# lhoyer/improving_segmentation_with_selfsupervised_depth

Measured on AMD Instinct MI355X. Metric: train images/sec, ResNet-101 joint seg+depth @512x1024, higher is better.
Workload: dtype f32

## Files before the change

improving_segmentation_with_selfsupervised_depth_amd/_lib.py:

```python
import ctypes
import os
from ctypes import c_int, c_long, c_float, c_void_p, c_size_t, c_uint64, c_int64, POINTER

_HERE = os.path.dirname(os.path.abspath(__file__))
LIB_PATH = os.environ.get("SEGSDE_LIB") or os.path.join(_HERE, "libsegsde_hip.so")
ABI_VERSION = 23

_LIB = None
HOST_POINTERS_OK = False


class PackJob(ctypes.Structure):
    _fields_ = [("w", c_void_p), ("fwd", c_void_p), ("dgrad", c_void_p)] + [(n, c_int) for n in (
        "O", "I", "KH", "KW", "block0", "reserved")]


class WinoJob(ctypes.Structure):
    _fields_ = [("w", c_void_p), ("u_fwd", c_void_p), ("u_dgrad", c_void_p)] + [(n, c_int) for n in ("O", "I", "block0", "reserved")]


class BnFoldJob(ctypes.Structure):
    _fields_ = [(n, c_void_p) for n in ("w", "cb", "gamma", "beta", "mean", "var", "w_out", "b_out")] + [("eps", c_float)] + [
        (n, c_int) for n in ("O", "I", "KH", "KW", "block0", "reserved")]


class ConvDesc(ctypes.Structure):
    _fields_ = [(n, c_int) for n in (
        "B", "H", "W", "C0", "C1", "ld0", "ld1", "up0", "Ho", "Wo", "Cout", "ldy", "ldy2", "nsplit",
        "KH", "KW", "stride", "dil", "pad", "pad_mode", "in_div", "act", "sum2x2", "accumulate", "compute")]
# ... 48 lines not shown
    "segsde_pack_weight_both": (c_int, [P, P, P, c_int, c_int, c_int, c_int, P]),
    "segsde_pack_weight_both_multi": (c_int, [P, c_int, c_int, P]),
    "segsde_reflect_dgrad_fix": (c_int, [P, c_int, P, P, c_int, P, c_int, c_int, c_int, c_int, c_int, c_int, c_int, P]),
    "segsde_bn_stats_workspace": (c_size_t, [c_long, c_int]),
    "segsde_bn_stats": (c_int, [P, c_int, c_long, c_int, P, P, P, P, c_float, c_float, P, P, c_size_t, P]),
    "segsde_bn_eval_stats": (c_int, [P, P, c_int, c_float, P, P, P]),
    "segsde_bn_fold": (c_int, [P, c_int, c_int, P]),
    "segsde_bn_apply": (c_int, [P, c_int, c_long, c_int, P, P, P, P, P, c_int, P, c_int, c_int, c_float, c_uint64, P]),
    "segsde_bn_backward_workspace": (c_size_t, [c_long, c_int]),
    "segsde_bn_backward": (c_int, [P, c_int, P, c_int, P, c_int, c_long, c_int, P, P, P, P, c_int, c_float, c_uint64, c_int,
                                   P, P, P, c_int, P, c_int, P, c_size_t, P]),
    "segsde_bn_mask_words": (c_size_t, [c_long, c_int]),
    "segsde_bn_apply_mask": (c_int, [P, c_int, c_long, c_int, P, P, P, P, P, c_int, P, c_int, c_int, c_float, c_uint64, P, P]),
    "segsde_bn_backward_mask": (c_int, [P, c_int, P, P, c_int, c_long, c_int, P, P, P, c_int, c_float, c_int, P, P, P, c_int, P, c_int,
                                        P, c_size_t, P]),
    "segsde_colsum_workspace": (c_size_t, [c_long, c_int]),
    "segsde_act_backward": (c_int, [P, c_int, P, c_int, c_long, c_int, c_int, P, c_int, P, P, c_size_t, P]),
    "segsde_colsum": (c_int, [P, c_int, c_long, c_int, P, P, c_size_t, P]),
    "segsde_feat_dist_workspace": (c_size_t, [c_long, c_int]),
    "segsde_feat_dist_forward": (c_int, [P, c_int, P, c_int, c_long, c_int, P, P, c_size_t, P]),
    "segsde_feat_dist_backward": (c_int, [P, c_int, P, c_int, c_long, c_int, P, P, P, c_int, P]),
    "segsde_maxpool3x3s2_forward": (c_int, [P, c_int, c_int, c_int, c_int, P, P, P]),
    "segsde_maxpool3x3s2_backward": (c_int, [P, P, c_int, c_int, c_int, c_int, P, c_int, P]),
    "segsde_upsample2x_backward": (c_int, [P, c_int, c_int, c_int, c_int, c_int, P, c_int, P]),
    "segsde_upsample2x_forward": (c_int, [P, c_int, c_int, c_int, c_int, c_int, P, c_int, P]),
    "segsde_resize_bilinear_forward": (c_int, [P, c_int, c_int, c_int, c_int, c_int, P, c_int, c_int, c_int, c_int, P]),
    "segsde_resize_bilinear_backward": (c_int, [P, c_int, c_int, c_int, c_int, c_int, P, c_int, c_int, c_int, c_int, P]),
    "segsde_global_avgpool_workspace": (c_size_t, [c_int, c_long, c_int]),
    "segsde_global_avgpool_forward": (c_int, [P, c_int, c_int, c_long, c_int, P, P, c_size_t, P]),
    "segsde_global_avgpool_backward": (c_int, [P, c_int, c_long, c_int, P, c_int, P]),
    "segsde_gate_forward": (c_int, [P, P, c_long, P, P]),
    "segsde_gate_backward": (c_int, [P, P, P, c_long, P, P, P]),
    "segsde_axpby": (c_int, [c_long, c_float, P, c_float, P, P, P]),
    "segsde_axpby_dev": (c_int, [c_long, P, P, P, P, P, P]),
    "segsde_scale_channels": (c_int, [P, c_int, c_int, c_long, c_int, P, P, c_int, P]),
    "segsde_dropout": (c_int, [P, c_int, c_long, c_int, c_float, c_uint64, P, c_int, P]),
    "segsde_copy_channels": (c_int, [P, c_int, P, c_int, c_long, c_int, P]),
    "segsde_nchw_to_nhwc": (c_int, [P, c_int, c_int, c_int, c_int, c_float, c_float, P, c_int, P]),
    "segsde_nhwc_to_nchw": (c_int, [P, c_int, c_int, c_int, c_int, c_int, P, P]),
    "segsde_pose_matrix_forward": (c_int, [P, P, c_int, c_int, c_int, P, P]),
    "segsde_pose_matrix_backward": (c_int, [P, P, P, c_int, c_int, c_int, P, P, P]),
    "segsde_warp_forward": (c_int, [P, c_int, c_int, P, P, P, P, c_int, c_int, c_int, c_float, c_float, P, P, P, P]),
    "segsde_warp_backward_workspace": (c_size_t, [c_int, c_int, c_int]),
    "segsde_warp_backward": (c_int, [P, P, c_int, c_int, P, P, P, P, c_int, c_int, c_int, c_float, c_float, P, P, P,
                                     c_size_t, P]),
    "segsde_reprojection_error_forward": (c_int, [P, P, c_int, c_int, c_int, c_int, P, c_long, P]),
# ... 99 lines not shown
```

improving_segmentation_with_selfsupervised_depth_amd/csrc/elementwise.hip:

```cpp
#include <stdlib.h>
#include "segsde_common.h"
#include <type_traits>
#include <utility>
#include <cstdlib>
#include <cstring>

namespace {

template <int VW> struct VecF { float v[VW]; };
template <int VW> __device__ __forceinline__ VecF<VW> ldv(const float* p) {
  VecF<VW> r;
  if (VW == 4) { const float4 t = *reinterpret_cast<const float4*>(p); r.v[0] = t.x; r.v[1 % VW] = t.y; r.v[2 % VW] = t.z; r.v[3 % VW] = t.w; }
  else r.v[0] = p[0];
  return r;
}
template <int VW> __device__ __forceinline__ void stv(float* p, const VecF<VW>& r) {
  if (VW == 4) *reinterpret_cast<float4*>(p) = make_float4(r.v[0], r.v[1 % VW], r.v[2 % VW], r.v[3 % VW]);
  else p[0] = r.v[0];
}

constexpr int SLAB = 64;
constexpr int RLANES = 4;

__host__ __device__ inline int red_blocks(long M) {
  long nb = (M + 255) / 256;
  return (int)(nb < 1 ? 1 : (nb > 512 ? 512 : nb));
}

template <class Op, int VW, class = void> struct has_ctx : std::false_type {};
template <class Op, int VW>
struct has_ctx<Op, VW, std::void_t<decltype(std::declval<const Op&>().template ctx<VW>(0))>> : std::true_type {};


template <class Op, int VW, int TX>
__global__ __launch_bounds__(256) void colreduce_kernel(Op op, long M, int C, double* part) {
  constexpr int TY = 256 / TX, CW = TX * VW;
  SEGSDE_SMEM;
  double* sh = reinterpret_cast<double*>(segsde_smem);
  const int tx = threadIdx.x % TX, ty = threadIdx.x / TX;
  const int c = blockIdx.y * CW + tx * VW;
  const int nb = gridDim.x;
  const long rows_per = (M + nb - 1) / nb;
  const long r_begin = blockIdx.x * rows_per;
  long r_end = r_begin + rows_per; if (r_end > M) r_end = M;
  double s0[VW], s1[VW];
#pragma unroll
  for (int j = 0; j < VW; ++j) { s0[j] = 0.0; s1[j] = 0.0; }
  if (c < C) {
    if constexpr (has_ctx<Op, VW>::value) {
      const auto k = op.template ctx<VW>(c);
      for (long m = r_begin + ty; m < r_end; m += TY) op.template row<VW>(m, c, k, s0, s1);
    } else {
#pragma unroll 4
      for (long m = r_begin + ty; m < r_end; m += TY) op.template row<VW>(m, c, s0, s1);
    }
  }
#pragma unroll
  for (int j = 0; j < VW; ++j) {
    sh[ty * CW + tx * VW + j] = s0[j];
    sh[(TY + ty) * CW + tx * VW + j] = s1[j];
  }
  __syncthreads();
  const int cc = threadIdx.x;
  if (cc < CW && blockIdx.y * CW + cc < C) {
    double a = 0.0, b2 = 0.0;
    for (int j = 0; j < TY; ++j) { a += sh[j * CW + cc]; b2 += sh[(TY + j) * CW + cc]; }
    part[((long)blockIdx.x * 2 + 0) * C + blockIdx.y * CW + cc] = a;
    part[((long)blockIdx.x * 2 + 1) * C + blockIdx.y * CW + cc] = b2;
  }
}

template <class Op, int TX>
void launch_colreduce_scalar(Op op, long M, int C, double* part, hipStream_t s) {
  const dim3 grid(red_blocks(M), (C + TX - 1) / TX);
// ... 373 lines not shown
    const int w = t % W; t /= W;
    const int h = t % H; const int b = t / H;
    float4 s = make_float4(0.f, 0.f, 0.f, 0.f);
    for (int kh = 0; kh < 3; ++kh) {
      const int hn = h + 1 - kh;
      if (hn < 0 || (hn & 1)) continue;
      const int ho = hn >> 1; if (ho >= Ho) continue;
      for (int kw = 0; kw < 3; ++kw) {
        const int wn = w + 1 - kw;
        if (wn < 0 || (wn & 1)) continue;
        const int wo = wn >> 1; if (wo >= Wo) continue;
        const long o = ((long)(b * Ho + ho) * Wo + wo) * C4 + c4;
        const uchar4 k = reinterpret_cast<const uchar4*>(idx)[o];
        const float4 g = reinterpret_cast<const float4*>(dy)[o];
        const unsigned char tap = (unsigned char)(kh * 3 + kw);
        s.x += k.x == tap ? g.x : 0.f; s.y += k.y == tap ? g.y : 0.f; s.z += k.z == tap ? g.z : 0.f; s.w += k.w == tap ? g.w : 0.f;
      }
    }
    if (accumulate) {
      const float4 o = reinterpret_cast<const float4*>(dx)[e];
      s.x += o.x; s.y += o.y; s.z += o.z; s.w += o.w;
    }
    reinterpret_cast<float4*>(dx)[e] = s;
  }
}

__global__ __launch_bounds__(256) void upsample2x_bwd_kernel(const float* dy, int lddy, int B, int h, int w, int C,
                                                             float* dx, int lddx) {
  const long total = (long)B * h * w * C;
  const int W2 = 2 * w;
  for (long e = blockIdx.x * 256L + threadIdx.x; e < total; e += (long)gridDim.x * 256) {
    const int c = (int)(e % C); long t = e / C;
    const int x = (int)(t % w); t /= w;
    const int y = (int)(t % h); const int b = (int)(t / h);
    const float* p = dy + ((long)(b * 2 * h + 2 * y) * W2 + 2 * x) * lddy + c;
    const float s = (p[0] + p[lddy]) + (p[(long)W2 * lddy] + p[(long)W2 * lddy + lddy]);
    dx[((long)(b * h + y) * w + x) * lddx + c] = s;
  }
}

__global__ __launch_bounds__(256) void upsample2x_fwd_kernel(const float* x, int ldx, int B, int h, int w, int C, float* y,
                                                             int ldy) {
  const long total = (long)B * 2 * h * 2 * w * C;
  for (long e = blockIdx.x * 256L + threadIdx.x; e < total; e += (long)gridDim.x * 256) {
    const int c = (int)(e % C); long t = e / C;
    const int X = (int)(t % (2 * w)); t /= 2 * w;
// ... 566 lines not shown
                       C / 4, Ho, Wo, y, idx);
  } else {
    hipLaunchKernelGGL(maxpool_fwd_kernel, dim3(ew_blocks((long)B * Ho * Wo * C)), dim3(256), 0, ST(stream), x, B, H, W, C,
                       Ho, Wo, y, idx);
  }
  SEGSDE_CHECK_LAUNCH();
  return 0;
}
extern "C" int segsde_maxpool3x3s2_backward(const float* dy, const uint8_t* idx, int B, int H, int W, int C, float* dx,
                                            int accumulate, void* stream) {
  if (!dy || !idx || !dx) return SEGSDE_ERR_NULL;
  const int Ho = (H - 1) / 2 + 1, Wo = (W - 1) / 2 + 1;
  if (C % 4 == 0 && (long)B * H * W * (C / 4) < (1L << 31) && al16p(dy) && al16p(dx) && (reinterpret_cast<uintptr_t>(idx) & 3) == 0) {
    hipLaunchKernelGGL(maxpool_bwd4_kernel, dim3(ew_blocks((long)B * H * W * (C / 4))), dim3(256), 0, ST(stream), dy, idx, B, H, W,
                       C / 4, Ho, Wo, dx, accumulate);
    SEGSDE_CHECK_LAUNCH();
    return 0;
  }
  hipLaunchKernelGGL(maxpool_bwd_kernel, dim3(ew_blocks((long)B * H * W * C)), dim3(256), 0, ST(stream), dy, idx, B, H, W,
                     C, Ho, Wo, dx, accumulate);
  SEGSDE_CHECK_LAUNCH();
  return 0;
}
extern "C" int segsde_upsample2x_backward(const float* dy, int lddy, int B, int h, int w, int C, float* dx, int lddx,
                                          void* stream) {
  if (!dy || !dx) return SEGSDE_ERR_NULL;
  hipLaunchKernelGGL(upsample2x_bwd_kernel, dim3(ew_blocks((long)B * h * w * C)), dim3(256), 0, ST(stream), dy, lddy, B, h,
                     w, C, dx, lddx);
  SEGSDE_CHECK_LAUNCH();
  return 0;
}
extern "C" int segsde_upsample2x_forward(const float* x, int ldx, int B, int h, int w, int C, float* y, int ldy, void* stream) {
  if (!x || !y) return SEGSDE_ERR_NULL;
  hipLaunchKernelGGL(upsample2x_fwd_kernel, dim3(ew_blocks((long)B * 4 * h * w * C)), dim3(256), 0, ST(stream), x, ldx, B, h, w, C,
                     y, ldy);
  SEGSDE_CHECK_LAUNCH();
  return 0;
}
extern "C" int segsde_resize_bilinear_forward(const float* x, int ldx, int B, int Hi, int Wi, int C, float* y, int ldy,
                                              int Ho, int Wo, int ac, void* stream) {
  if (!x || !y) return SEGSDE_ERR_NULL;
  hipLaunchKernelGGL(resize_fwd_kernel, dim3(ew_blocks((long)B * Ho * Wo * C)), dim3(256), 0, ST(stream), x, ldx, B, Hi, Wi,
                     C, y, ldy, Ho, Wo, ac);
  SEGSDE_CHECK_LAUNCH();
  return 0;
}
// ... 135 lines not shown
```

improving_segmentation_with_selfsupervised_depth_amd/functional.py:

```python
import collections
import weakref

import torch
from torch.autograd import Function as _TorchFunction

from . import hipops as H


class Function(_TorchFunction):

    @classmethod
    def apply(cls, *args):
        return super(_TorchFunction, cls).apply(*args)


FUSIONS = {}
BN_BITMASK = True


def _grad_dest(param):
    from . import ddp
    return ddp.grad_destination(param) if ddp._GRAD_DEST else None


# ... 584 lines not shown


class MaxPoolFn(Function):

    @staticmethod
    def forward(ctx, x, box=None):
        y, idx = H.maxpool_forward(_c(x))
        ctx.shape = tuple(x.shape)
        ctx.box = box
        ctx.save_for_backward(idx)
        return y

    @staticmethod
    def backward(ctx, dy):
        (idx,) = ctx.saved_tensors
        box = ctx.box
        acc = box.get("g") if (box is not None and box.get("fused")) else None
        dx = H.maxpool_backward(_c(dy), idx, ctx.shape, accumulate_into=acc)
        if box is not None and acc is None and box.get("publish") and box.get("g") is None:
            box["g"], box["fused"] = dx, True
        return dx, None


class ResizeFn(Function):
    @staticmethod
    def forward(ctx, x, out_hw, align_corners):
        ctx.in_hw, ctx.ac = (x.shape[1], x.shape[2]), align_corners
        return H.resize_bilinear(x, out_hw, align_corners)

    @staticmethod
    def backward(ctx, dy):
        return H.resize_bilinear_backward(_c(dy), ctx.in_hw, ctx.ac), None, None


def resize_bilinear(x_nhwc, out_hw, align_corners=False):
    out_hw = (int(out_hw[0]), int(out_hw[1]))
    if not align_corners and out_hw == (x_nhwc.shape[1], x_nhwc.shape[2]):
        return x_nhwc
    return ResizeFn.apply(x_nhwc, out_hw, align_corners)


class GlobalAvgPoolFn(Function):
    @staticmethod
    def forward(ctx, x):
        ctx.shape = tuple(x.shape)
        return H.global_avgpool(x)
# ... 137 lines not shown
```

improving_segmentation_with_selfsupervised_depth_amd/hipops.py:

```python
import ctypes
import os
import threading

import numpy as np
import torch

from . import _lib
from ._lib import ConvDesc, check

ACT = {"none": 0, "relu": 1, "elu": 2, "sigmoid": 3}


class _Slot(threading.local):

    def __init__(self, default=None):
        self.default = default
        self.v = default

    def __getattr__(self, name):
        if name == "v":
            return self.__dict__.setdefault("v", self.__dict__.get("default"))
        raise AttributeError(name)

    def __getitem__(self, i):
# ... 987 lines not shown
    return da

def maxpool_forward(x):
    B, H, W, C = x.shape
    x = x.contiguous()
    Ho, Wo = (H - 1) // 2 + 1, (W - 1) // 2 + 1
    y = torch.empty((B, Ho, Wo, C), dtype=torch.float32, device=x.device)
    idx = torch.empty((B, Ho, Wo, C), dtype=torch.uint8, device=x.device)
    _timed('hbm_maxpool_fwd', 4.0 * x.numel() * 1.25 + 0.25 * x.numel(), x, lambda: check(_lib.lib().segsde_maxpool3x3s2_forward(_p(_f32(x)), B, H, W, C, _p(y), _p(idx), _stream(x)), "maxpool_fwd"))
    return y, idx


def maxpool_backward(dy, idx, in_shape, accumulate_into=None):
    B, H, W, C = in_shape
    dy = dy.contiguous()
    acc = accumulate_into if (accumulate_into is not None and tuple(accumulate_into.shape) == tuple(in_shape)
                              and accumulate_into.is_contiguous()) else None
    dx = acc if acc is not None else torch.empty(in_shape, dtype=torch.float32, device=dy.device)
    check(_lib.lib().segsde_maxpool3x3s2_backward(_p(_f32(dy)), _p(idx), B, H, W, C, _p(dx), 1 if acc is not None else 0,
                                                  _stream(dy)), "maxpool_bwd")
    return dx


def resize_bilinear(x, out_hw, align_corners=False):
    B, Hi, Wi, C = x.shape
    Ho, Wo = out_hw
    y = torch.empty((B, Ho, Wo, C), dtype=torch.float32, device=x.device)
    check(_lib.lib().segsde_resize_bilinear_forward(_p(_f32(x)), nhwc_ld(x), B, Hi, Wi, C, _p(y), C, Ho, Wo,
                                                    int(align_corners), _stream(x)), "resize_fwd")
    return y


def resize_bilinear_backward(dy, in_hw, align_corners=False):
    B, Ho, Wo, C = dy.shape
    Hi, Wi = in_hw
    dx = torch.empty((B, Hi, Wi, C), dtype=torch.float32, device=dy.device)
    check(_lib.lib().segsde_resize_bilinear_backward(_p(_f32(dy)), nhwc_ld(dy), B, Hi, Wi, C, _p(dx), C, Ho, Wo,
                                                     int(align_corners), _stream(dy)), "resize_bwd")
    return dx


def global_avgpool(x):
    B, H, W, C = x.shape
    y = torch.empty((B, 1, 1, C), dtype=torch.float32, device=x.device)
    L = _lib.lib()
    nws = int(L.segsde_global_avgpool_workspace(B, H * W, C))
# ... 987 lines not shown
```

improving_segmentation_with_selfsupervised_depth_amd/models/joint_segmentation_depth.py:

```python
import torch
from torch import nn

from .. import functional as Fn
from .joint_segmentation_depth_decoder import JointSegDepthDecoder, PAD
from .utils import get_depth_decoder, get_posenet, get_resnet_backbone


class JointSegmentationMonodepth(nn.Module):
    def __init__(self, models, frame_ids, use_pose_net, num_pose_frames, provide_uncropped_for_pose):
        super().__init__()
        self.frame_ids = frame_ids
        self.use_pose_net = use_pose_net
        self.num_pose_frames = num_pose_frames
        self.provide_uncropped_for_pose = provide_uncropped_for_pose
        self.device = torch.device("cuda" if torch.cuda.is_available() else "cpu")
        self.models = nn.ModuleDict(models)
        from .depth_decoder import DepthDecoder
        dec = [m for k, v in self.models.items() if k in ("depth", "segmentation", "mtl_decoder")
               for m in v.modules() if isinstance(m, DepthDecoder) and m.use_skips and m.takes_fan_views()]
        if "encoder" in self.models:
            self.models["encoder"].skip_consumers = len(dec)
        import os
        self.defer_trunk_backward = os.environ.get("SEGSDE_DEFER_TRUNK", "0") not in ("", "0")

    def _run_pose_nets(self, frames):
        return self.models["pose"]([self.models["pose_encoder"](frames)])

    def predict_poses(self, inputs, features):
        key = "color_full_aug" if self.provide_uncropped_for_pose else "color_aug"
        frame = lambda f: inputs[key, f, 0]
        temporal = [(slot, f) for slot, f in enumerate(self.frame_ids[1:]) if f != "s"]
        outputs = {}

        def emit(f, axisangle, translation, column, invert):
            outputs[("axisangle", 0, f)] = axisangle
            outputs[("translation", 0, f)] = translation
            outputs[("cam_T_cam", 0, f)] = Fn.PoseMatrixFn.apply(axisangle[:, column:column + 1], translation[:, column:column + 1], invert)

        if self.num_pose_frames == 2:
            for _, f in temporal:
                first, second = (f, 0) if f < 0 else (0, f)
                emit(f, *self._run_pose_nets(torch.cat([frame(first), frame(second)], 1)), 0, f < 0)
        else:
            both = self._run_pose_nets(torch.cat([frame(f) for f in self.frame_ids if f != "s"], 1))
# ... 77 lines not shown
```

improving_segmentation_with_selfsupervised_depth_amd/models/layers.py:

```python
import os

import torch
from torch import nn

from .. import functional as Fn
from .. import hipops as H
from ..hipops import ConvGeom


def _seed():
    return int(torch.randint(0, 2 ** 31 - 1, (1,)).item())


_NO_FUSED_STATS = bool(int(os.environ.get("SEGSDE_NO_FUSED_STATS", "0")))


GRAPH_SAFE_DROPOUT = [False]
_PACK_SCOPE = [0, 0]


class weight_pack_scope:

    def __init__(self, model=None):
        self._model = model
# ... 104 lines not shown
                self._stats_wanted = False
                return Fn.ConvFn.apply(x, skip, weight, self.bias, g, act, None, grad_box, packs, x0_act, None, None, wc)
            if not self._stats_offered:
                self._stats_offered = True
            holder = []
            y = Fn.ConvFn.apply(x, skip, weight, self.bias, g, act, holder, grad_box, packs, x0_act, None, None, wc)
            y._bn_partials = (holder[0], y._version, self) if holder and holder[0] is not None else None
            return y
        if act == "none":
            return Fn.ConvFn.apply(x, skip, weight, self.bias, g, act, None, grad_box, packs, x0_act, None, None, wc)
        box = {"need_dbias": self.bias is not None and self.bias.requires_grad}
        fc = self._fold_cache
        fc["want"] = (_PACK_SCOPE[0], weight._version, weight.data_ptr(), weight.device, c0) if (_PACK_SCOPE[0] and up) else None
        yz = Fn.ConvFn.apply(x, skip, weight, self.bias, g, act, None, grad_box, packs, x0_act, box, fc, wc, skip_box)
        if not (torch.is_grad_enabled() and yz.requires_grad):
            return yz
        y = Fn.ActGradFn.apply(yz, act, box)
        y._preact = (yz, act, y._version)
        return y


class BatchNorm2d(nn.BatchNorm2d):

    def forward(self, x, residual=None, act="none", drop_p=0.0, grad_box=None):
        training = self.training or (self.running_mean is None)
        nbt = self.num_batches_tracked if (self.training and self.track_running_stats
                                           and self.num_batches_tracked is not None) else None
        if self.momentum is None:
            momentum = 1.0 / float(int(self.num_batches_tracked) + 1) if nbt is not None else 0.0
        else:
            momentum = self.momentum
        if drop_p > 0 and GRAPH_SAFE_DROPOUT[0]:
            y = self.forward(x, residual, act, 0.0, grad_box)
            return torch.nn.functional.dropout(y, drop_p, True)
        seed = _seed() if drop_p > 0 else 0
        partials = getattr(x, "_bn_partials", None) if training else None
        if partials is not None:
            partials, version, producer = partials
            if partials.shape[-1] != self.num_features or x._version != version:
                partials = None
            elif producer._stats_wanted is not True:
                producer._stats_wanted = True
        if training:
            Fn.fusion("bn_stats_from_conv_epilogue", partials is not None)
        return Fn.BNActFn.apply(x, self.weight, self.bias, residual, self.running_mean, self.running_var, training,
                                momentum, self.eps, act, drop_p, seed, partials, grad_box, nbt)


def _tensor_key(t):
    return None if t is None else (t._version, t.data_ptr(), t.device)


def _folded(conv, bn):
    key = (id(bn), float(bn.eps)) + tuple(_tensor_key(t) for t in (conv.weight, conv.bias, bn.weight, bn.bias, bn.running_mean,
                                                                     bn.running_var))
    e = conv.__dict__["_bn_fold"]
    if e.get("key") != key:
        w, b = H.bn_fold(conv.weight, conv.bias, bn.weight, bn.bias, bn.running_mean, bn.running_var, bn.eps)
        e.clear()
        e.update(key=key, w=w, b=b)
    return e


def drop_folded(model):
    for m in model.modules():
        if isinstance(m, Conv2d):
            m._bn_fold.clear()


# ... 16 lines not shown
        return None
    kn = H.winograd_fused_ok(g, B, Hh, W)
    wino = kn or H.winograd_ok(g, B, Hh, W)
    e = _folded(conv, bn)
    pk = ("pack", c0)
    if pk not in e:
        w = e["w"]
        if c0 > conv.in_channels:
            w = torch.nn.functional.pad(w, (0, 0, 0, 0, 0, c0 - conv.in_channels))
        e[pk] = H.pack_weight(w, False)
    if residual is not None:
        if residual.stride(-1) != 1:
            residual = Fn._c(residual)
        return H.conv_forward(g, x, None, e[pk], e["b"], act, residual=residual)
    wino_f = None
    if wino:
        wk = ("wino", bool(kn))
        if wk not in e:
            e[wk] = H.winograd_pack(e["w"], kn=bool(kn))[0]
        wino_f = e[wk]
    return H.conv_forward(g, x, None, e[pk], e["b"], act, wino=wino_f)


def conv_bn(conv, bn, x, residual=None, act="none", drop_p=0.0, bn_grad_box=None, image_norm=None, **conv_kwargs):
    if Fn.FROZEN_BN_FOLD[0]:
        ok = (not torch.is_grad_enabled() and not bn.training and bn.running_mean is not None and bn.running_var is not None
              and not drop_p > 0 and not conv_kwargs.get("up") and conv_kwargs.get("skip") is None
              and conv_kwargs.get("act", "none") == "none")
        y = _folded_forward(conv, bn, x, residual, act, image_norm) if ok else None
        Fn.fusion("frozen_bn_folded", y is not None)
        if y is not None:
            return y
    if image_norm is not None:
        y0 = conv.forward_image(x, *image_norm)
        if y0 is None:
            y0 = conv(Fn.to_nhwc(x, image_norm[0], image_norm[1], pad_to=4), **conv_kwargs)
    else:
        y0 = conv(x, **conv_kwargs)
    return bn(y0, residual=residual, act=act, drop_p=drop_p, grad_box=bn_grad_box)
```

improving_segmentation_with_selfsupervised_depth_amd/models/resnet_encoder.py:

```python
import errno
import os

import numpy as np
import torch
from torch import nn

from .. import functional as Fn
from .layers import Conv2d, BatchNorm2d, conv_bn


class BasicBlock(nn.Module):
    expansion = 1

    def __init__(self, inplanes, planes, stride=1, downsample=None, dilation=1):
        super().__init__()
        if dilation > 1:
            raise NotImplementedError("Dilation > 1 not supported in BasicBlock")
        self.conv1 = Conv2d(inplanes, planes, 3, stride, 1, bias=False)
        self.bn1 = BatchNorm2d(planes)
        self.relu = nn.ReLU(inplace=True)
        self.conv2 = Conv2d(planes, planes, 3, 1, 1, bias=False)
        self.bn2 = BatchNorm2d(planes)
        self.downsample = downsample

# ... 109 lines not shown
        load_imnet_weights(model, num_layers, num_input_images)
    return model


class ResnetEncoder(nn.Module):

    def __init__(self, num_layers, pretrained, num_input_images=1, **kwargs):
        super().__init__()
        self.num_ch_enc = np.array([64, 64, 128, 256, 512])
        if num_layers not in _SPECS:
            raise ValueError("{} is not a valid number of resnet layers".format(num_layers))
        if num_input_images > 1:
            self.encoder = resnet_multiimage_input(num_layers, pretrained, num_input_images)
        else:
            block, layers = _SPECS[num_layers]
            self.encoder = ResNet(block, layers, 1, kwargs.get("replace_stride_with_dilation"))
            if pretrained:
                load_imnet_weights(self.encoder, num_layers)
        if num_layers > 34:
            self.num_ch_enc[1:] *= 4

    def forward_nhwc(self, input_image):
        e = self.encoder
        f0 = conv_bn(e.conv1, e.bn1, input_image, act="relu", image_norm=(0.45, 0.225))
        feats = [f0]
        n_dec = int(getattr(self, "skip_consumers", 0))
        defer = bool(getattr(self, "defer_backward", False)) and torch.is_grad_enabled()
        n = 1 if defer else n_dec
        Fn.release_fans(id(self))
        (x0,), box0 = Fn.fan_feature(f0, n, 1, owner=id(self))
        x = Fn.MaxPoolFn.apply(x0, box0)
        layers = (e.layer1, e.layer2, e.layer3, e.layer4)
        x_ds, box = None, None
        for li, layer in enumerate(layers):
            for bi, blk in enumerate(layer):
                x = blk(x, x_ds, box) if (bi == 0 and x_ds is not None) else blk(x)
            feats.append(x)
            x_ds, box = None, None
            if li + 1 < len(layers) and n > 0 and layers[li + 1][0].downsample is not None:
                (x, x_ds), box = Fn.fan_feature(x, n, 2, owner=id(self))
                if box is None:
                    x_ds = None
        if defer:
            feats = Fn.defer_trunk(feats, id(self), n_dec)
        return feats

    def forward(self, input_image):
        self.features = [Fn.to_nchw(f) for f in self.forward_nhwc(input_image)]
        return self.features
```

include/segsde_hip.h:

```cpp
#ifndef SEGSDE_HIP_H
#define SEGSDE_HIP_H
#include <stddef.h>
#include <stdint.h>

#ifdef __cplusplus
extern "C" {
#endif

#define SEGSDE_ABI_VERSION 23

enum { SEGSDE_ERR_NULL = -1, SEGSDE_ERR_SHAPE = -2, SEGSDE_ERR_WORKSPACE = -3, SEGSDE_ERR_UNSUPPORTED = -4 };
enum { SEGSDE_ACT_NONE = 0, SEGSDE_ACT_RELU = 1, SEGSDE_ACT_ELU = 2, SEGSDE_ACT_SIGMOID = 3 };
enum { SEGSDE_DTYPE_F32 = 0, SEGSDE_DTYPE_I64 = 1, SEGSDE_DTYPE_U8 = 2 };
enum { SEGSDE_PAD_ZERO = 0, SEGSDE_PAD_REFLECT = 1, SEGSDE_PAD_REFLECT_ADJOINT = 2 };

int segsde_abi_version(void);

typedef struct segsde_conv_desc {
  int B, H, W;
  int C0, C1;
  int ld0, ld1;
  int up0;
  int Ho, Wo, Cout;
  int ldy, ldy2, nsplit;
  int KH, KW, stride, dil, pad;
  int pad_mode;
  int in_div;
  int act;
  int sum2x2;
  int accumulate;
  int compute;
} segsde_conv_desc;
// ... 77 lines not shown
size_t segsde_bn_mask_words(long M, int C);
int segsde_bn_apply_mask(const float* x, int ldx, long M, int C, const float* mean, const float* invstd, const float* gamma,
                         const float* beta, const float* residual, int ldr, float* y, int ldy, int act, float drop_p,
                         uint64_t seed, uint32_t* mask, void* stream);
int segsde_bn_backward_mask(const float* dy, int lddy, const uint32_t* mask, const float* x, int ldx, long M, int C,
                            const float* mean, const float* invstd, const float* gamma, int act, float drop_p,
                            int batch_stats, float* dgamma, float* dbeta, float* dx, int lddx, float* dres, int lddres,
                            void* workspace, size_t workspace_bytes, void* stream);
size_t segsde_colsum_workspace(long M, int C);
int segsde_act_backward(const float* dy, int lddy, const float* y, int ldy, long M, int C, int act, float* dz, int lddz,
                        float* dbias, void* workspace, size_t workspace_bytes, void* stream);
int segsde_colsum(const float* x, int ldx, long M, int C, float* out, void* workspace, size_t workspace_bytes,
                  void* stream);

size_t segsde_feat_dist_workspace(long M, int C);
int segsde_feat_dist_forward(const float* a, int lda, const float* b, int ldb, long M, int C, float* dist, void* workspace,
                             size_t workspace_bytes, void* stream);
int segsde_feat_dist_backward(const float* a, int lda, const float* b, int ldb, long M, int C, const float* dist,
                              const float* grad, float* da, int ldda, void* stream);

int segsde_maxpool3x3s2_forward(const float* x, int B, int H, int W, int C, float* y, uint8_t* idx, void* stream);
int segsde_maxpool3x3s2_backward(const float* dy, const uint8_t* idx, int B, int H, int W, int C, float* dx, int accumulate,
                                 void* stream);
int segsde_upsample2x_backward(const float* dy, int lddy, int B, int h, int w, int C, float* dx, int lddx, void* stream);
int segsde_upsample2x_forward(const float* x, int ldx, int B, int h, int w, int C, float* y, int ldy, void* stream);
int segsde_resize_bilinear_forward(const float* x, int ldx, int B, int Hi, int Wi, int C, float* y, int ldy, int Ho, int Wo,
                                   int align_corners, void* stream);
int segsde_resize_bilinear_backward(const float* dy, int lddy, int B, int Hi, int Wi, int C, float* dx, int lddx, int Ho,
                                    int Wo, int align_corners, void* stream);
size_t segsde_global_avgpool_workspace(int B, long HW, int C);
int segsde_global_avgpool_forward(const float* x, int ldx, int B, long HW, int C, float* y, void* ws, size_t ws_bytes,
                                  void* stream);
int segsde_global_avgpool_backward(const float* dy, int B, long HW, int C, float* dx, int lddx, void* stream);
int segsde_gate_forward(const float* f, const float* a, long n, float* y, void* stream);
int segsde_gate_backward(const float* dy, const float* f, const float* a, long n, float* df, float* da, void* stream);
int segsde_axpby(long n, float alpha, const float* x, float beta, const float* y, float* out, void* stream);
int segsde_axpby_dev(long n, const float* alpha, const float* x, const float* beta, const float* y, float* out, void* stream);
int segsde_copy_channels(const float* src, int lds, float* dst, int ldd, long M, int C, void* stream);
int segsde_scale_channels(const float* x, int ldx, int B, long HW, int C, const float* scale, float* y, int ldy, void* stream);
int segsde_dropout(const float* x, int ldx, long M, int C, float p, uint64_t seed, float* y, int ldy, void* stream);
int segsde_nchw_to_nhwc(const float* x, int B, int C, int H, int W, float mean, float std, float* y, int ldy, void* stream);
int segsde_nchw_to_nhwc_bordered(const float* x, int B, int C, int H, int W, float mean, float sd, float* y, int ldy, int pad_top,
                                 int pad_left, int Hp, int Wp, void* stream);
int segsde_nhwc_to_nchw(const float* x, int ldx, int B, int C, int H, int W, float* y, void* stream);

typedef struct segsde_wino_job {
// ... 192 lines not shown
```

Measured before the change: 64.07.

## Fuse stem BN+ReLU+maxpool forward and backward for pose encoder

Adds HIP kernels that apply batch-norm, ReLU and 3x3 stride-2 maxpool in one pass, plus a fused backward that gathers pooled gradients while reducing BN statistics and computing dx. The pose encoder no longer keeps its full-resolution stem feature, so the large activation tensor is not written and then reread. This trades extra recomputation of the BN/ReLU in backward and a gather-heavy reduction kernel for lower memory traffic and fewer launches.

```diff
diff --git a/improving_segmentation_with_selfsupervised_depth_amd/_lib.py b/improving_segmentation_with_selfsupervised_depth_amd/_lib.py
--- a/improving_segmentation_with_selfsupervised_depth_amd/_lib.py
+++ b/improving_segmentation_with_selfsupervised_depth_amd/_lib.py
@@ -4,7 +4,7 @@
 
 _HERE = os.path.dirname(os.path.abspath(__file__))
 LIB_PATH = os.environ.get("SEGSDE_LIB") or os.path.join(_HERE, "libsegsde_hip.so")
-ABI_VERSION = 23
+ABI_VERSION = 24
 
 _LIB = None
 HOST_POINTERS_OK = False
@@ -99,6 +99,9 @@
     "segsde_feat_dist_backward": (c_int, [P, c_int, P, c_int, c_long, c_int, P, P, P, c_int, P]),
     "segsde_maxpool3x3s2_forward": (c_int, [P, c_int, c_int, c_int, c_int, P, P, P]),
     "segsde_maxpool3x3s2_backward": (c_int, [P, P, c_int, c_int, c_int, c_int, P, c_int, P]),
+    "segsde_bn_apply_maxpool": (c_int, [P, c_int, c_int, c_int, c_int, c_int, P, P, P, P, P, P, P, c_int, P]),
+    "segsde_bn_backward_maxpool": (c_int, [P, P, P, c_int, P, c_int, c_int, c_int, c_int, c_int, P, P, P, P, P, P, P, c_int, P, c_size_t,
+                                           P]),
     "segsde_upsample2x_backward": (c_int, [P, c_int, c_int, c_int, c_int, c_int, P, c_int, P]),
     "segsde_upsample2x_forward": (c_int, [P, c_int, c_int, c_int, c_int, c_int, P, c_int, P]),
     "segsde_resize_bilinear_forward": (c_int, [P, c_int, c_int, c_int, c_int, c_int, P, c_int, c_int, c_int, c_int, P]),
diff --git a/improving_segmentation_with_selfsupervised_depth_amd/csrc/elementwise.hip b/improving_segmentation_with_selfsupervised_depth_amd/csrc/elementwise.hip
--- a/improving_segmentation_with_selfsupervised_depth_amd/csrc/elementwise.hip
+++ b/improving_segmentation_with_selfsupervised_depth_amd/csrc/elementwise.hip
@@ -31,6 +31,10 @@
 template <class Op, int VW>
 struct has_ctx<Op, VW, std::void_t<decltype(std::declval<const Op&>().template ctx<VW>(0))>> : std::true_type {};
 
+
+template <class Op> struct row_unroll { static constexpr int value = 1; };
+struct BnPoolBwdOp;
+template <> struct row_unroll<BnPoolBwdOp> { static constexpr int value = 4; };
 
 template <class Op, int VW, int TX>
 __global__ __launch_bounds__(256) void colreduce_kernel(Op op, long M, int C, double* part) {
@@ -49,7 +53,12 @@
   if (c < C) {
     if constexpr (has_ctx<Op, VW>::value) {
       const auto k = op.template ctx<VW>(c);
-      for (long m = r_begin + ty; m < r_end; m += TY) op.template row<VW>(m, c, k, s0, s1);
+      if constexpr (row_unroll<Op>::value > 1) {
+#pragma unroll(row_unroll<Op>::value)
+        for (long m = r_begin + ty; m < r_end; m += TY) op.template row<VW>(m, c, k, s0, s1);
+      } else {
+        for (long m = r_begin + ty; m < r_end; m += TY) op.template row<VW>(m, c, k, s0, s1);
+      }
     } else {
 #pragma unroll 4
       for (long m = r_begin + ty; m < r_end; m += TY) op.template row<VW>(m, c, s0, s1);
@@ -469,6 +478,148 @@
       s.x += o.x; s.y += o.y; s.z += o.z; s.w += o.w;
     }
     reinterpret_cast<float4*>(dx)[e] = s;
+  }
+}
+
+__global__ __launch_bounds__(256) void bn_apply_maxpool4_kernel(const float* x, int ldx, int B, int H, int W, int C4, int Ho, int Wo,
+                                                                const float* mean, const float* invstd, const float* gamma,
+                                                                const float* beta, float* y, uint8_t* idx, float* act, int ldact) {
+  const long total = (long)B * Ho * Wo * C4;
+  for (long e = blockIdx.x * 256L + threadIdx.x; e < total; e += (long)gridDim.x * 256) {
+    const int c4 = (int)(e % C4); long t = e / C4;
+    const int wo = (int)(t % Wo); t /= Wo;
+    const int ho = (int)(t % Ho); const int b = (int)(t / Ho);
+    const int c = c4 * 4;
+    const VecF<4> mu = ldv<4>(mean + c), is = ldv<4>(invstd + c);
+    VecF<4> ga, be;
+    if (gamma) { ga = ldv<4>(gamma + c); be = ldv<4>(beta + c); }
+    float best[4] = {-INFINITY, -INFINITY, -INFINITY, -INFINITY};
+    int bi[4] = {0, 0, 0, 0};
+    bool first = true;
+    for (int kh = 0; kh < 3; ++kh) {
+      const int h = 2 * ho - 1 + kh;
+      if (h < 0 || h >= H) continue;
+      for (int kw = 0; kw < 3; ++kw) {
+        const int w = 2 * wo - 1 + kw;
+        if (w < 0 || w >= W) continue;
+        const long m = (long)(b * H + h) * W + w;
+        const VecF<4> xv = ldv<4>(x + m * ldx + c);
+        VecF<4> v;
+#pragma unroll
+        for (int j = 0; j < 4; ++j) {
+          float tt = (xv.v[j] - mu.v[j]) * is.v[j];
+          if (gamma) tt = tt * ga.v[j] + be.v[j];
+          v.v[j] = segsde_act(tt, SEGSDE_ACT_RELU);
+        }
+        if (act && kh >= 1 && kw >= 1) stv<4>(act + m * ldact + c, v);
+#pragma unroll
+        for (int j = 0; j < 4; ++j)
+          if (first || v.v[j] > best[j] || v.v[j] != v.v[j]) { best[j] = v.v[j]; bi[j] = kh * 3 + kw; }
+        first = false;
+      }
+    }
+    reinterpret_cast<float4*>(y)[e] = make_float4(best[0], best[1], best[2], best[3]);
+    reinterpret_cast<uchar4*>(idx)[e] = make_uchar4((unsigned char)bi[0], (unsigned char)bi[1], (unsigned char)bi[2], (unsigned char)bi[3]);
+  }
+}
+
+struct PoolGrad {
+  const float* dy; const uint8_t* idx; const float* extra; int ldextra; int H, W, C4, Ho, Wo, w_shift, h_shift;
+  __device__ __forceinline__ VecF<4> quad(long m, int c) const {
+    int w, h, b;
+    if (w_shift >= 0 && h_shift >= 0) {
+      w = (int)(m & (W - 1)); const int t = (int)(m >> w_shift); h = t & (H - 1); b = t >> h_shift;
+    } else {
+      const int mi = (int)m; w = mi % W; const int t = mi / W; h = t % H; b = t / H;
+    }
+    const int oh = h & 1, ow = w & 1;
+    const int ho0 = (h + oh) >> 1, kh0 = oh ? 0 : 1, ho1 = (h - 1) >> 1;
+    const int wo0 = (w + ow) >> 1, kw0 = ow ? 0 : 1, wo1 = (w - 1) >> 1;
+    const bool vh0 = ho0 < Ho, vh1 = oh != 0, vw0 = wo0 < Wo, vw1 = ow != 0;
+    const int hos[2] = {vh0 ? ho0 : 0, vh1 ? ho1 : 0}, wos[2] = {vw0 ? wo0 : 0, vw1 ? wo1 : 0};
+    const int khs[2] = {kh0, 2}, kws[2] = {kw0, 2};
+    const bool vhs[2] = {vh0, vh1}, vws[2] = {vw0, vw1};
+    uchar4 k[4]; float4 g[4];
+#pragma unroll
+    for (int a = 0; a < 2; ++a)
+#pragma unroll
+      for (int d = 0; d < 2; ++d) {
+        const long o = ((long)(b * Ho + hos[a]) * Wo + wos[d]) * C4 + (c >> 2);
+        k[a * 2 + d] = reinterpret_cast<const uchar4*>(idx)[o];
+        g[a * 2 + d] = reinterpret_cast<const float4*>(dy)[o];
+      }
+    float4 s = make_float4(0.f, 0.f, 0.f, 0.f);
+#pragma unroll
+    for (int a = 0; a < 2; ++a)
+#pragma unroll
+      for (int d = 0; d < 2; ++d) {
+        const bool ok = vhs[a] && vws[d];
+        const unsigned char tap = (unsigned char)(khs[a] * 3 + kws[d]);
+        const uchar4 kk = k[a * 2 + d]; const float4 gg = g[a * 2 + d];
+        s.x += ok && kk.x == tap ? gg.x : 0.f; s.y += ok && kk.y == tap ? gg.y : 0.f;
+        s.z += ok && kk.z == tap ? gg.z : 0.f; s.w += ok && kk.w == tap ? gg.w : 0.f;
+      }
+    if (extra) {
+      const float4 o = *reinterpret_cast<const float4*>(extra + m * ldextra + c);
+      s.x += o.x; s.y += o.y; s.z += o.z; s.w += o.w;
+    }
+    VecF<4> r; r.v[0] = s.x; r.v[1] = s.y; r.v[2] = s.z; r.v[3] = s.w;
+    return r;
+  }
+};
+
+struct BnPoolBwdOp {
+  PoolGrad pg; const float* x; int ldx; const float* mean; const float* invstd; const float* gamma; const float* beta;
+  template <int VW> struct Ctx { VecF<VW> mu, is, ga, be; };
+  template <int VW> __device__ Ctx<VW> ctx(int c) const {
+    Ctx<VW> k;
+    k.mu = ldv<VW>(mean + c); k.is = ldv<VW>(invstd + c);
+    if (gamma) { k.ga = ldv<VW>(gamma + c); k.be = ldv<VW>(beta + c); }
+    return k;
+  }
+  template <int VW> __device__ void row(long m, int c, const Ctx<VW>& k, double* s0, double* s1) const {
+    static_assert(VW == 4, "the pooled gradient is gathered per channel quad");
+    const VecF<4> g = pg.quad(m, c), xx = ldv<4>(x + m * ldx + c);
+#pragma unroll
+    for (int j = 0; j < 4; ++j) {
+      const float xh = (xx.v[j] - k.mu.v[j]) * k.is.v[j];
+      const float dz = bn_dz_remask(g.v[j], xh, gamma ? k.ga.v[j] : 1.f, gamma ? k.be.v[j] : 0.f, gamma != nullptr, SEGSDE_ACT_RELU);
+      s0[j] += (double)dz * (double)xh; s1[j] += (double)dz;
+    }
+  }
+};
+
+__global__ __launch_bounds__(256) void bn_pool_bwd_apply_kernel(PoolGrad pg, const float* x, int ldx, long M, int C, const float* mean,
+                                                                const float* invstd, const float* gamma, const float* beta,
+                                                                const float* dgamma, const float* dbeta, float* dx, int lddx,
+                                                                int cv_shift) {
+  const int CV = C / 4;
+  const long total = M * CV;
+  const float invM = 1.f / (float)M;
+  const long stride = (long)gridDim.x * 256;
+  const bool fixed_c = cv_shift >= 0 && (stride & (long)(CV - 1)) == 0;
+  VecF<4> ga, be, mu, is, dg, db;
+  auto load_params = [&](int c) {
+    is = ldv<4>(invstd + c); mu = ldv<4>(mean + c);
+    if (gamma) { ga = ldv<4>(gamma + c); be = ldv<4>(beta + c); }
+    dg = ldv<4>(dgamma + c); db = ldv<4>(dbeta + c);
+  };
+  if (fixed_c) load_params((int)((blockIdx.x * 256L + threadIdx.x) & (long)(CV - 1)) * 4);
+  for (long e = blockIdx.x * 256L + threadIdx.x; e < total; e += stride) {
+    const long m = cv_shift >= 0 ? (e >> cv_shift) : e / CV;
+    const int c = (int)(e - m * CV) * 4;
+    const VecF<4> g = pg.quad(m, c), xx = ldv<4>(x + m * ldx + c);
+    if (!fixed_c) load_params(c);
+    VecF<4> o;
+#pragma unroll
+    for (int j = 0; j < 4; ++j) {
+      const float dz = bn_dz_remask(g.v[j], (xx.v[j] - mu.v[j]) * is.v[j], gamma ? ga.v[j] : 1.f, gamma ? be.v[j] : 0.f, gamma != nullptr,
+                                    SEGSDE_ACT_RELU);
+      const float gm = gamma ? ga.v[j] : 1.f;
+      const float xh = (xx.v[j] - mu.v[j]) * is.v[j];
+      o.v[j] = gm * is.v[j] * (dz - db.v[j] * invM - xh * dg.v[j] * invM);
+    }
+    stv<4>(dx + m * lddx + c, o);
   }
 }
 
@@ -1081,6 +1232,53 @@
   SEGSDE_CHECK_LAUNCH();
   return 0;
 }
+
+extern "C" int segsde_bn_apply_maxpool(const float* x, int ldx, int B, int H, int W, int C, const float* mean, const float* invstd,
+                                       const float* gamma, const float* beta, float* y, uint8_t* idx, float* act, int ldact,
+                                       void* stream) {
+  if (!x || !mean || !invstd || !y || !idx) return SEGSDE_ERR_NULL;
+  if ((gamma == nullptr) != (beta == nullptr)) return SEGSDE_ERR_NULL;
+  if (B <= 0 || H <= 0 || W <= 0 || C <= 0 || ldx < C || (act && ldact < C)) return SEGSDE_ERR_SHAPE;
+  const bool v4 = (C % 4 == 0) && (ldx % 4 == 0) && al16(x) && al16(y) && (reinterpret_cast<uintptr_t>(idx) & 3) == 0 &&
+                  al16(mean) && al16(invstd) && (!gamma || (al16(gamma) && al16(beta))) && (!act || ((ldact % 4 == 0) && al16(act))) &&
+                  (long)B * H * W < (1L << 31);
+  if (!v4) return SEGSDE_ERR_UNSUPPORTED;
+  const int Ho = (H - 1) / 2 + 1, Wo = (W - 1) / 2 + 1;
+  hipLaunchKernelGGL(bn_apply_maxpool4_kernel, dim3(ew_blocks((long)B * Ho * Wo * (C / 4))), dim3(256), 0, ST(stream), x, ldx, B, H, W,
+                     C / 4, Ho, Wo, mean, invstd, gamma, beta, y, idx, act, ldact);
+  SEGSDE_CHECK_LAUNCH();
+  return 0;
+}
+
+extern "C" int segsde_bn_backward_maxpool(const float* dy, const uint8_t* idx, const float* extra, int ldextra, const float* x, int ldx,
+                                          int B, int H, int W, int C, const float* mean, const float* invstd, const float* gamma,
+                                          const float* beta, float* dgamma, float* dbeta, float* dx, int lddx, void* ws,
+                                          size_t ws_bytes, void* stream) {
+  if (!dy || !idx || !x || !mean || !invstd || !dgamma || !dbeta || !ws) return SEGSDE_ERR_NULL;
+  if ((gamma == nullptr) != (beta == nullptr)) return SEGSDE_ERR_NULL;
+  if (B <= 0 || H <= 0 || W <= 0 || C <= 0 || ldx < C || (extra && ldextra < C) || (dx && lddx < C)) return SEGSDE_ERR_SHAPE;
+  const long M = (long)B * H * W;
+  const bool v4 = (C % 4 == 0) && (ldx % 4 == 0) && al16p(x) && al16p(dy) && (reinterpret_cast<uintptr_t>(idx) & 3) == 0 &&
+                  (!extra || ((ldextra % 4 == 0) && al16p(extra))) && (!gamma || (al16p(gamma) && al16p(beta))) && al16p(mean) &&
+                  al16p(invstd) && (!dx || ((lddx % 4 == 0) && al16p(dx))) && al16p(dgamma) && al16p(dbeta) && M * (C / 4) < (1L << 31);
+  if (!v4) return SEGSDE_ERR_UNSUPPORTED;
+  if (ws_bytes < part_bytes(M, C)) return SEGSDE_ERR_WORKSPACE;
+  const int Ho = (H - 1) / 2 + 1, Wo = (W - 1) / 2 + 1;
+  const PoolGrad pg{dy, idx, extra, ldextra, H, W, C / 4, Ho, Wo, pow2_shift(W), pow2_shift(H)};
+  BnPoolBwdOp op{pg, x, ldx, mean, invstd, gamma, beta};
+  hipLaunchKernelGGL((colreduce_kernel<BnPoolBwdOp, 4, SLAB / 4>), dim3(red_blocks(M), (C + SLAB - 1) / SLAB), dim3(256),
+                     2 * 16 * SLAB * sizeof(double), ST(stream), op, M, C, (double*)ws);
+  SEGSDE_CHECK_LAUNCH();
+  hipLaunchKernelGGL(pair_finalize_kernel, dim3((C + 15) / 16), dim3(256), 4096, ST(stream), (const double*)ws,
+                     red_blocks(M), C, dgamma, dbeta);
+  SEGSDE_CHECK_LAUNCH();
+  if (dx) {
+    hipLaunchKernelGGL(bn_pool_bwd_apply_kernel, dim3(ew_blocks_cv(M * C / 4, C / 4)), dim3(256), 0, ST(stream), pg, x, ldx, M, C, mean,
+                       invstd, gamma, beta, (const float*)dgamma, (const float*)dbeta, dx, lddx, pow2_shift(C / 4));
+    SEGSDE_CHECK_LAUNCH();
+  }
+  return 0;
+}
 extern "C" int segsde_upsample2x_backward(const float* dy, int lddy, int B, int h, int w, int C, float* dx, int lddx,
                                           void* stream) {
   if (!dy || !dx) return SEGSDE_ERR_NULL;
diff --git a/improving_segmentation_with_selfsupervised_depth_amd/functional.py b/improving_segmentation_with_selfsupervised_depth_amd/functional.py
--- a/improving_segmentation_with_selfsupervised_depth_amd/functional.py
+++ b/improving_segmentation_with_selfsupervised_depth_amd/functional.py
@@ -630,6 +630,51 @@
         return dx, None
 
 
+STEM_POOL_FUSION = True
+
+
+class BNReluPoolFn(Function):
+
+    @staticmethod
+    def forward(ctx, x, gamma, beta, running_mean, running_var, momentum, eps, partials=None, nbt=None):
+        x = _c(x)
+        if partials is not None:
+            mean, invstd = H.bn_stats_from_partials(partials, x.numel() // x.shape[-1], running_mean, running_var, momentum,
+                                                    eps, update_running=running_mean is not None, num_batches_tracked=nbt)
+        else:
+            mean, invstd = H.bn_stats(x, running_mean, running_var, momentum, eps, update_running=running_mean is not None,
+                                      num_batches_tracked=nbt)
+        r = H.bn_apply_maxpool(x, mean, invstd, gamma, beta) if x.dim() == 4 else None
+        ctx.fused = r is not None
+        fusion("stem_bn_relu_pool", ctx.fused)
+        if r is None:
+            y, idx = H.maxpool_forward(H.bn_apply(x, mean, invstd, gamma, beta, None, "relu"))
+        else:
+            y, idx = r[0], r[1]
+        ctx.beta_param = beta
+        ctx.save_for_backward(x, gamma, beta, mean, invstd, idx)
+        return y
+
+    @staticmethod
+    def backward(ctx, dy):
+        x, gamma, beta, mean, invstd, idx = ctx.saved_tensors
+        want_g = gamma is not None and ctx.needs_input_grad[1]
+        bp = ctx.beta_param
+        dests = dict(dgamma_out=_grad_dest(gamma) if want_g else None,
+                     dbeta_out=_grad_dest(bp) if (want_g and bp is not None and ctx.needs_input_grad[2]) else None)
+        ctx.beta_param = None
+        r = H.bn_backward_maxpool(_c(dy), idx, x, mean, invstd, gamma, beta, need_dx=ctx.needs_input_grad[0], **dests) if ctx.fused else None
+        if r is None:
+            g = H.maxpool_backward(_c(dy), idx, tuple(x.shape))
+            dx, _, dgamma, dbeta = H.bn_backward(g, None, x, mean, invstd, gamma, "relu", batch_stats=True,
+                                                 need_dx=ctx.needs_input_grad[0], beta=beta, **dests)
+        else:
+            dx, dgamma, dbeta = r
+        if not want_g:
+            dgamma = dbeta = None
+        return dx, dgamma, dbeta, None, None, None, None, None, None
+
+
 class ResizeFn(Function):
     @staticmethod
     def forward(ctx, x, out_hw, align_corners):
diff --git a/improving_segmentation_with_selfsupervised_depth_amd/hipops.py b/improving_segmentation_with_selfsupervised_depth_amd/hipops.py
--- a/improving_segmentation_with_selfsupervised_depth_amd/hipops.py
+++ b/improving_segmentation_with_selfsupervised_depth_amd/hipops.py
@@ -1033,6 +1033,47 @@
     return dx
 
 
+def bn_apply_maxpool(x, mean, invstd, gamma, beta, keep_act=False):
+    B, H, W, C = x.shape
+    ld = nhwc_ld(x)
+    Ho, Wo = (H - 1) // 2 + 1, (W - 1) // 2 + 1
+    y = torch.empty((B, Ho, Wo, C), dtype=torch.float32, device=x.device)
+    idx = torch.empty((B, Ho, Wo, C), dtype=torch.uint8, device=x.device)
+    act = torch.empty((B, H, W, C), dtype=torch.float32, device=x.device) if keep_act else None
+    n = x.numel()
+    code = _timed('hbm_bn_apply_maxpool', (4.0 + 1.0 + 0.0625 + (4.0 if keep_act else 0.0)) * n, x,
+                  lambda: _lib.lib().segsde_bn_apply_maxpool(_p(_f32(x)), ld, B, H, W, C, _p(mean), _p(invstd), _p(gamma), _p(beta), _p(y),
+                                                             _p(idx), _p(act), C, _stream(x)))
+    if code == -4:
+        return None
+    check(code, "bn_apply_maxpool")
+    return y, idx, act
+
+
+def bn_backward_maxpool(dy, idx, x, mean, invstd, gamma, beta, extra=None, need_dx=True, dgamma_out=None, dbeta_out=None):
+    B, H, W, C = x.shape
+    M, ldx = B * H * W, nhwc_ld(x)
+    L = _lib.lib()
+    dy = dy.contiguous()
+
+    def _dst(t):
+        ok = t is not None and tuple(t.shape) == (C,) and t.is_contiguous() and t.dtype == torch.float32
+        return t if ok else torch.empty(C, dtype=torch.float32, device=x.device)
+    dgamma, dbeta = _dst(dgamma_out), _dst(dbeta_out)
+    dx = torch.empty(x.shape, dtype=torch.float32, device=x.device) if need_dx else None
+    nb = L.segsde_bn_backward_workspace(M, C)
+    ws = _ws(nb, x)
+    per_pass = 4.0 + 1.0 + 0.0625 + (4.0 if extra is not None else 0.0)
+    code = _timed('hbm_bn_backward_maxpool', (2.0 * per_pass + (4.0 if need_dx else 0.0)) * M * C, x,
+                  lambda: L.segsde_bn_backward_maxpool(_p(_f32(dy)), _p(idx), _p(extra), nhwc_ld(extra) if extra is not None else 0,
+                                                       _p(_f32(x)), ldx, B, H, W, C, _p(mean), _p(invstd), _p(gamma), _p(beta),
+                                                       _p(dgamma), _p(dbeta), _p(dx), C, _p(ws), nb, _stream(x)))
+    if code == -4:
+        return None
+    check(code, "bn_backward_maxpool")
+    return dx, dgamma, dbeta
+
+
 def resize_bilinear(x, out_hw, align_corners=False):
     B, Hi, Wi, C = x.shape
     Ho, Wo = out_hw
diff --git a/improving_segmentation_with_selfsupervised_depth_amd/models/joint_segmentation_depth.py b/improving_segmentation_with_selfsupervised_depth_amd/models/joint_segmentation_depth.py
--- a/improving_segmentation_with_selfsupervised_depth_amd/models/joint_segmentation_depth.py
+++ b/improving_segmentation_with_selfsupervised_depth_amd/models/joint_segmentation_depth.py
@@ -20,6 +20,8 @@
                for m in v.modules() if isinstance(m, DepthDecoder) and m.use_skips and m.takes_fan_views()]
         if "encoder" in self.models:
             self.models["encoder"].skip_consumers = len(dec)
+        if "pose_encoder" in self.models:
+            self.models["pose_encoder"].keep_feature0 = False
         import os
         self.defer_trunk_backward = os.environ.get("SEGSDE_DEFER_TRUNK", "0") not in ("", "0")
 
diff --git a/improving_segmentation_with_selfsupervised_depth_amd/models/layers.py b/improving_segmentation_with_selfsupervised_depth_amd/models/layers.py
--- a/improving_segmentation_with_selfsupervised_depth_amd/models/layers.py
+++ b/improving_segmentation_with_selfsupervised_depth_amd/models/layers.py
@@ -150,7 +150,7 @@
 
 class BatchNorm2d(nn.BatchNorm2d):
 
-    def forward(self, x, residual=None, act="none", drop_p=0.0, grad_box=None):
+    def _step_args(self):
         training = self.training or (self.running_mean is None)
         nbt = self.num_batches_tracked if (self.training and self.track_running_stats
                                            and self.num_batches_tracked is not None) else None
@@ -158,21 +158,37 @@
             momentum = 1.0 / float(int(self.num_batches_tracked) + 1) if nbt is not None else 0.0
         else:
             momentum = self.momentum
-        if drop_p > 0 and GRAPH_SAFE_DROPOUT[0]:
-            y = self.forward(x, residual, act, 0.0, grad_box)
-            return torch.nn.functional.dropout(y, drop_p, True)
-        seed = _seed() if drop_p > 0 else 0
-        partials = getattr(x, "_bn_partials", None) if training else None
+        return training, nbt, momentum
+
+    def _conv_partials(self, x):
+        partials = getattr(x, "_bn_partials", None)
         if partials is not None:
             partials, version, producer = partials
             if partials.shape[-1] != self.num_features or x._version != version:
                 partials = None
             elif producer._stats_wanted is not True:
                 producer._stats_wanted = True
+        return partials
+
+    def forward(self, x, residual=None, act="none", drop_p=0.0, grad_box=None):
+        training, nbt, momentum = self._step_args()
+        if drop_p > 0 and GRAPH_SAFE_DROPOUT[0]:
+            y = self.forward(x, residual, act, 0.0, grad_box)
+            return torch.nn.functional.dropout(y, drop_p, True)
+        seed = _seed() if drop_p > 0 else 0
+        partials = self._conv_partials(x) if training else None
         if training:
             Fn.fusion("bn_stats_from_conv_epilogue", partials is not None)
         return Fn.BNActFn.apply(x, self.weight, self.bias, residual, self.running_mean, self.running_var, training,
                                 momentum, self.eps, act, drop_p, seed, partials, grad_box, nbt)
+
+    def forward_relu_pool(self, x):
+        training, nbt, momentum = self._step_args()
+        if not (training and Fn.STEM_POOL_FUSION):
+            return Fn.MaxPoolFn.apply(self.forward(x, act="relu"))
+        partials = self._conv_partials(x)
+        Fn.fusion("bn_stats_from_conv_epilogue", partials is not None)
+        return Fn.BNReluPoolFn.apply(x, self.weight, self.bias, self.running_mean, self.running_var, momentum, self.eps, partials, nbt)
 
 
 def _tensor_key(t):
@@ -235,7 +251,7 @@
     return H.conv_forward(g, x, None, e[pk], e["b"], act, wino=wino_f)
 
 
-def conv_bn(conv, bn, x, residual=None, act="none", drop_p=0.0, bn_grad_box=None, image_norm=None, **conv_kwargs):
+def conv_bn(conv, bn, x, residual=None, act="none", drop_p=0.0, bn_grad_box=None, image_norm=None, pool=False, **conv_kwargs):
     if Fn.FROZEN_BN_FOLD[0]:
         ok = (not torch.is_grad_enabled() and not bn.training and bn.running_mean is not None and bn.running_var is not None
               and not drop_p > 0 and not conv_kwargs.get("up") and conv_kwargs.get("skip") is None
@@ -243,11 +259,14 @@
         y = _folded_forward(conv, bn, x, residual, act, image_norm) if ok else None
         Fn.fusion("frozen_bn_folded", y is not None)
         if y is not None:
-            return y
+            return Fn.MaxPoolFn.apply(y) if pool else y
     if image_norm is not None:
         y0 = conv.forward_image(x, *image_norm)
         if y0 is None:
             y0 = conv(Fn.to_nhwc(x, image_norm[0], image_norm[1], pad_to=4), **conv_kwargs)
     else:
         y0 = conv(x, **conv_kwargs)
+    if pool:
+        assert act == "relu" and residual is None and not drop_p > 0 and bn_grad_box is None
+        return bn.forward_relu_pool(y0)
     return bn(y0, residual=residual, act=act, drop_p=drop_p, grad_box=bn_grad_box)
diff --git a/improving_segmentation_with_selfsupervised_depth_amd/models/resnet_encoder.py b/improving_segmentation_with_selfsupervised_depth_amd/models/resnet_encoder.py
--- a/improving_segmentation_with_selfsupervised_depth_amd/models/resnet_encoder.py
+++ b/improving_segmentation_with_selfsupervised_depth_amd/models/resnet_encoder.py
@@ -155,14 +155,18 @@
 
     def forward_nhwc(self, input_image):
         e = self.encoder
-        f0 = conv_bn(e.conv1, e.bn1, input_image, act="relu", image_norm=(0.45, 0.225))
-        feats = [f0]
         n_dec = int(getattr(self, "skip_consumers", 0))
         defer = bool(getattr(self, "defer_backward", False)) and torch.is_grad_enabled()
         n = 1 if defer else n_dec
         Fn.release_fans(id(self))
-        (x0,), box0 = Fn.fan_feature(f0, n, 1, owner=id(self))
-        x = Fn.MaxPoolFn.apply(x0, box0)
+        if n == 0 and not getattr(self, "keep_feature0", True):
+            feats = [None]
+            x = conv_bn(e.conv1, e.bn1, input_image, act="relu", image_norm=(0.45, 0.225), pool=True)
+        else:
+            f0 = conv_bn(e.conv1, e.bn1, input_image, act="relu", image_norm=(0.45, 0.225))
+            feats = [f0]
+            (x0,), box0 = Fn.fan_feature(f0, n, 1, owner=id(self))
+            x = Fn.MaxPoolFn.apply(x0, box0)
         layers = (e.layer1, e.layer2, e.layer3, e.layer4)
         x_ds, box = None, None
         for li, layer in enumerate(layers):
@@ -179,5 +183,5 @@
         return feats
 
     def forward(self, input_image):
-        self.features = [Fn.to_nchw(f) for f in self.forward_nhwc(input_image)]
+        self.features = [None if f is None else Fn.to_nchw(f) for f in self.forward_nhwc(input_image)]
         return self.features
diff --git a/include/segsde_hip.h b/include/segsde_hip.h
--- a/include/segsde_hip.h
+++ b/include/segsde_hip.h
@@ -7,7 +7,7 @@
 extern "C" {
 #endif
 
-#define SEGSDE_ABI_VERSION 23
+#define SEGSDE_ABI_VERSION 24
 
 enum { SEGSDE_ERR_NULL = -1, SEGSDE_ERR_SHAPE = -2, SEGSDE_ERR_WORKSPACE = -3, SEGSDE_ERR_UNSUPPORTED = -4 };
 enum { SEGSDE_ACT_NONE = 0, SEGSDE_ACT_RELU = 1, SEGSDE_ACT_ELU = 2, SEGSDE_ACT_SIGMOID = 3 };
@@ -131,6 +131,12 @@
 int segsde_maxpool3x3s2_forward(const float* x, int B, int H, int W, int C, float* y, uint8_t* idx, void* stream);
 int segsde_maxpool3x3s2_backward(const float* dy, const uint8_t* idx, int B, int H, int W, int C, float* dx, int accumulate,
                                  void* stream);
+int segsde_bn_apply_maxpool(const float* x, int ldx, int B, int H, int W, int C, const float* mean, const float* invstd,
+                            const float* gamma, const float* beta, float* y, uint8_t* idx, float* act, int ldact, void* stream);
+int segsde_bn_backward_maxpool(const float* dy, const uint8_t* idx, const float* extra, int ldextra, const float* x, int ldx, int B,
+                               int H, int W, int C, const float* mean, const float* invstd, const float* gamma, const float* beta,
+                               float* dgamma, float* dbeta, float* dx, int lddx, void* workspace, size_t workspace_bytes,
+                               void* stream);
 int segsde_upsample2x_backward(const float* dy, int lddy, int B, int h, int w, int C, float* dx, int lddx, void* stream);
 int segsde_upsample2x_forward(const float* x, int ldx, int B, int h, int w, int C, float* y, int ldy, void* stream);
 int segsde_resize_bilinear_forward(const float* x, int ldx, int B, int Hi, int Wi, int C, float* y, int ldy, int Ho, int Wo,
```

New measurement: 64.34, median of 6. No clear change (+0.4%).
